# Yoshiki172/Deep-Learning-based-RGBA-Image-Compression-with-Masked-Window-based-Attention

Measured on AMD Instinct MI355X. Metric: MPixels/sec encode+decode, 256×256 RGBA batch; bpp & PSNR parity vs reference, higher is better.
Workload: dtype bf16; 1 GPU; AutoEncoderRGB_Journal forward encode+decode (BASELINE config 2), 256x256 RGBA; global_batch=8, per_gpu_batch=8, height=256, width=256, parallelism=replicas1, hip_graph=True, tile_cache=profiles/tune_fwd_bf16_b8_256.json

## Files before the change

### deep-learning-based-rgba-image-compression-with-masked-window-based-attention_amd/csrc/conv.hip

```cpp
#include <cstdio>
#include <cstdlib>
#include <utility>

#include "common.h"
#include "conv_common.h"

namespace rgbac {

#ifdef RGBAC_WG_TIMING
__device__ unsigned long long g_wg_t[16384][4];
#define WG_T(k)                                                                              \
  do {                                                                                       \
    if (threadIdx.x == 0) {                                                                  \
      const unsigned b_ = blockIdx.x + gridDim.x * (blockIdx.y + gridDim.y * blockIdx.z);    \
      if (b_ < 16384) g_wg_t[b_][k] = wall_clock64();                                        \
    }                                                                                        \
  } while (0)
#else
#define WG_T(k) do {} while (0)
#endif

template <typename T, int BM, int BN, int WGM, int WGN, int NBUF, int KSM = 1>
__global__ void __launch_bounds__(256) conv_kernel(const ConvArgsDev args) {
  constexpr int EPV = Elem<T>::EPV;
// ... 1935 lines not shown
#pragma unroll
          for (int r = 0; r < 4; ++r) v[j][r] += t[r];
        }
    }
#pragma unroll
    for (int j = 0; j < TN; ++j)
      if (nn[j] < cout) Elem<T>::st4(out + opix * ldo + nn[j], v[j]);
  }
}

template <int TN, int TM, bool DACT>
__device__ __forceinline__ void patch_epilogue(const ConvShared& s, const ConvGroup& g, int ph,
                                               int b, int yrow0, int x0, int fr,
                                               const int (&nn)[TN], const f32x4 (&acc)[TN][TM],
                                               const float (*pbias)[4] = nullptr) {
  const bool lean = s.mode != RGBAC_SUBPEL2 && !g.zout && !g.res1 && (g.cout & 3) == 0;
  if (lean && s.act == RGBAC_ACT_NONE) {
    patch_epi<TN, TM, RGBAC_ACT_NONE>(s, g, ph, b, yrow0, x0 + fr, nn, acc, pbias);
  } else if (lean && s.act == RGBAC_ACT_GELU) {
    patch_epi<TN, TM, RGBAC_ACT_GELU>(s, g, ph, b, yrow0, x0 + fr, nn, acc, pbias);
  } else if (lean && s.act == RGBAC_ACT_RELU) {
    patch_epi<TN, TM, RGBAC_ACT_RELU>(s, g, ph, b, yrow0, x0 + fr, nn, acc, pbias);
  } else if (DACT && lean && is_dact(s.act)) {
    patch_epi<TN, TM, RGBAC_ACT_DGELU>(s, g, ph, b, yrow0, x0 + fr, nn, acc, pbias);
  } else {
#pragma unroll
    for (int i = 0; i < TM; ++i) {
      const int m = (b * s.Hm + yrow0 + i) * s.Wm + x0 + fr;
      epilogue_tile_row<bf16_t, TN, TM, DACT>(s, g, ph, m, nn, acc, i);
    }
  }
}

template <int TH, int BN, int WGM, int WGN, int NBUF, bool DACT>
__global__ void __launch_bounds__(512) conv_patch_kernel(const ConvArgsDev args) {
  using T = bf16_t;
  constexpr int NW = 8;
  static_assert(WGM * WGN == NW, "8 waves");
  constexpr int TW = 16, PW = TW + 2, PH = TH + 2, PR = PH * PW;
  constexpr int RSC = 10;
  constexpr int PPIECE = (PR * RSC + 63) / 64;
  constexpr int PQ = (PPIECE + NW - 1) / NW;
  constexpr int TM = TH / WGM, TN = BN / WGN / 16;
  static_assert(TM >= 1 && TN >= 1 && TM * WGM == TH && TN * WGN * 16 == BN, "tile");
  constexpr int IA = BN / 8;
  constexpr int NAW = (IA + NW - 1) / NW;
  static_assert(NBUF == 3 || NBUF == 4, "ring depth (the patch rider sits at tap NBUF-1 of "
                                        "a group; groups have >= 4 taps)");
  constexpr int RT = NBUF - 1;
  constexpr int WSTAGE = BN * 8;
  constexpr int PSTAGE = PPIECE * 64;
  __shared__ __attribute__((aligned(16))) uint4 smem[NBUF * WSTAGE + 2 * PSTAGE];

  const ConvShared& s = args.s;
  const int tid = threadIdx.x, lane = tid & 63;
  const int wave = __builtin_amdgcn_readfirstlane(tid >> 6);
  const int txn = s.Wm / TW, tyn = s.Hm / TH;
  int nblk, txi, tyi, b, gi;
  {
    const int nwg = gridDim.x * gridDim.y;
    int t = blockIdx.x + gridDim.x * blockIdx.y;
    if (s.remap) {
      const int xcd = t & 7, q = nwg >> 3, r = nwg & 7;
      t = (xcd < r ? xcd * (q + 1) : r * (q + 1) + (xcd - r) * q) + (t >> 3);
    }
    nblk = t % gridDim.y; t /= gridDim.y;
    txi = t % txn; t /= txn;
// ... 153 lines not shown
    __builtin_amdgcn_s_barrier();
    __builtin_amdgcn_sched_barrier(0);
    if (it + NBUF - 1 < ns) STAGE_ISSUE(it + NBUF - 1);
    const uint4* As = smem + (it % NBUF) * WSTAGE;
    const uint4* Ps = smem + NBUF * WSTAGE + (cgrp & 1) * PSTAGE + toff;
#pragma unroll
    for (int ks = 0; ks < 2; ++ks) {
      uint4 a[TN], bb[TM];
#pragma unroll
      for (int j = 0; j < TN; ++j) a[j] = As[(ks ? a1 : a0) + j * 128];
#pragma unroll
      for (int i = 0; i < TM; ++i) bb[i] = Ps[bbase[i] + 4 * ks];
#pragma unroll
      for (int j = 0; j < TN; ++j)
#pragma unroll
        for (int i = 0; i < TM; ++i) mma_step<T>(acc[j][i], a[j], bb[i]);
    }
    ++ctap;
    if (++ctx == ctw) {
      ctx = 0;
      toff += convt ? (-PW + ctw - 1) * RSC : (PW - ctw + 1) * RSC;
    } else {
      toff += convt ? -RSC : RSC;
    }
    if (ctap == cntap) {
      ctap = 0; ctx = 0; ++cgrp;
      toff = convt ? (2 * PW + 2) * RSC : 0;
      if (++cck == nck) {
        cck = 0;
        if (!s2 || cph == 3 || pz >= 0) {
          int nn[TN];
#pragma unroll
          for (int j = 0; j < TN; ++j) nn[j] = n0 + wn * TN * 16 + j * 16 + fq * 4;
          if (s2 && pz >= 0) {
#pragma unroll
            for (int i = 0; i < TM; ++i) {
              const int m = (b * s.Hm + y0 + wm * TM + i) * s.Wm + x0 + fr;
#pragma unroll
              for (int j = 0; j < TN; ++j)
                if (nn[j] < g.cout)
                  *reinterpret_cast<float4*>(g.ws + ((size_t)pz * s.M + m) * g.cout16 + nn[j]) =
                      make_float4(acc[j][i][0], acc[j][i][1], acc[j][i][2], acc[j][i][3]);
            }
          } else {
            patch_epilogue<TN, TM, DACT>(s, g, s2 ? 0 : cph, b, y0 + wm * TM, x0, fr, nn, acc);
          }
#pragma unroll
          for (int j = 0; j < TN; ++j)
#pragma unroll
            for (int i = 0; i < TM; ++i) acc[j][i] = f32x4{0.f, 0.f, 0.f, 0.f};
        }
        ++cph;
        ctw = 3 - (cph & 1);
        cntap = (3 - (cph >> 1)) * ctw;
      }
    }
  }
#undef STAGE_ISSUE
#undef PATCH_ISSUE
}

template <int TH, int BN, int NW, int R, int CPT = 0, int KS = 1>
__global__ void __launch_bounds__(64 * NW * KS) conv_fpatch_kernel(const ConvArgsDev args) {
  using T = bf16_t;
  constexpr int TW = 16, PW = TW + 2, PR = (TH + 2) * PW;
  constexpr int TM = TH, TN = BN / NW / 16;
  static_assert(TN * NW * 16 == BN, "tile");
// ... 715 lines not shown
  if (tile < 0 || tile >= kNumTiles) return -1;
  return (fpatch_tile(tile) || kTiles[tile].kind == kNPatch) ? 1 : 0;
}
extern "C" int rgbac_conv_max_groups(void) { return kMaxGroups; }

extern "C" int rgbac_conv2d_grouped_describe(const rgbac_conv_args* args, int ngroups,
                                             char* kernel, int cap) {
  ConvArgsDev d;
  ConvPlan p;
  const int rc = plan_conv(args, ngroups, false, d, p);
  if (rc == RGBAC_OK && kernel && cap > 0) snprintf(kernel, (size_t)cap, "%s", p.name);
  return rc;
}

extern "C" int rgbac_conv2d_grouped(const rgbac_conv_args* args, int ngroups, void* stream) {
  return rgbac_conv2d_grouped_part(args, ngroups, 0, stream);
}

extern "C" int rgbac_conv2d_grouped_part(const rgbac_conv_args* args, int ngroups, int part,
                                         void* stream) {
  RGBAC_REQUIRE(part >= 0 && part <= 2, "part must be 0 (all), 1 (main) or 2 (split-K epilogue)");
  ConvArgsDev d;
  ConvPlan p;
  const int rc = plan_conv(args, ngroups, true, d, p);
  if (rc) return rc;
  hipStream_t st = reinterpret_cast<hipStream_t>(stream);
  if (args[0].dtype == RGBAC_F32) return launch_conv<float>(d, p, st, part);
  return launch_conv<bf16_t>(d, p, st, part);
}

extern "C" int rgbac_conv2d(const rgbac_conv_args* a, void* stream) {
  return rgbac_conv2d_grouped(a, 1, stream);
}
```

### deep-learning-based-rgba-image-compression-with-masked-window-based-attention_amd/csrc/conv_common.h

```cpp
#pragma once
#include "common.h"

namespace rgbac {

constexpr int kMaxGroups = 10;

struct ConvGroup {
  const void* sp0; const void* sp1; const void* sp2;
  long long sld0, sld1, sld2;
  const void* w;
  const float* bias;
  void* out;
  const void* res0; const void* res1; const void* res2;
  long long ld0, ld1, ld2, out_ldc;
  const uint8_t* sel;
  float* ws;
  const float* aux0;
  float* aux1;
  double* partial;
  void* zout;
  long long zld;
  int* cnt;
  int send0, send1, send2;
  int cin_pad, k_pad, cout, rows, cout16, out_coff;
// ... 374 lines not shown
    }
  }
}

template <typename T>
__device__ __forceinline__ float gauss_elem(const ConvGroup& g, int m, int c, int nch, float mu,
                                            float sg) {
  const float yv = Elem<T>::ld(reinterpret_cast<const T*>(g.res1) + (long long)m * g.ld1 + c);
  const float hat = rintf(yv - mu) + mu;
  Elem<T>::st(reinterpret_cast<T*>(g.out) + (long long)m * g.out_ldc + g.out_coff + c, hat);
  const float xin = g.aux0 ? yv + g.aux0[(long long)m * nch + c] : hat;
  const float v = fabsf(xin - mu);
  const float sc = fmaxf(sg, 0.11f);
  const float lik = fmaxf(std_cum_f((0.5f - v) / sc) - std_cum_f((-0.5f - v) / sc), 1e-9f);
  if (g.aux1) g.aux1[(long long)m * nch + c] = lik;
  const float bits = (-1.0f * logf(lik + 1e-10f)) / 0.69314718055994530942f;
  return fminf(fmaxf(bits, 0.0f), 50.0f);
}

template <typename T>
__device__ __forceinline__ float gauss_elem_y(const ConvGroup& g, int m, int c, int nch, float mu,
                                              float sg, float yv) {
  const float hat = rintf(yv - mu) + mu;
  Elem<T>::st(reinterpret_cast<T*>(g.out) + (long long)m * g.out_ldc + g.out_coff + c, hat);
  const float xin = g.aux0 ? yv + g.aux0[(long long)m * nch + c] : hat;
  const float v = fabsf(xin - mu);
  const float sc = fmaxf(sg, 0.11f);
  const float lik = fmaxf(std_cum_f((0.5f - v) / sc) - std_cum_f((-0.5f - v) / sc), 1e-9f);
  if (g.aux1) g.aux1[(long long)m * nch + c] = lik;
  const float bits = (-1.0f * logf(lik + 1e-10f)) / 0.69314718055994530942f;
  return fminf(fmaxf(bits, 0.0f), 50.0f);
}

bool pw3_ok(const ConvArgsDev& d, int cin_max);
void launch_pw3(const ConvArgsDev& d, hipStream_t st);

typedef __attribute__((address_space(3))) void* lptr_t;

__device__ __forceinline__ void dma16(const void* src, uint4* lds_block) {
  const uint32_t lds = __builtin_amdgcn_readfirstlane((uint32_t)(size_t)(lptr_t)lds_block);
  uint32_t keep;
  asm volatile(
      "s_mov_b32 %0, m0\n\t"
      "s_mov_b32 m0, %2\n\t"
      "s_nop 0\n\t"
      "global_load_lds_dwordx4 %1, off\n\t"
      "s_mov_b32 m0, %0"
      : "=&s"(keep)
      : "v"(src), "s"(lds)
      : "memory");
}

__device__ __forceinline__ void dma16_s(const void* sbase, uint32_t voff, uint32_t lds) {
  uint32_t keep;
  asm volatile(
      "s_mov_b32 %0, m0\n\t"
      "s_mov_b32 m0, %3\n\t"
      "s_nop 0\n\t"
      "global_load_lds_dwordx4 %1, %2\n\t"
      "s_mov_b32 m0, %0"
      : "=&s"(keep)
      : "v"(voff), "s"(sbase), "s"(lds)
      : "memory");
}
__device__ __forceinline__ void dma16_l(const void* src, uint32_t lds) {
  uint32_t keep;
// ... 31 lines not shown
```

### deep-learning-based-rgba-image-compression-with-masked-window-based-attention_amd/rgbac/_lib.py

```python
import ctypes
import os

import torch

_HERE = os.path.dirname(os.path.abspath(__file__))
LIB_PATH = os.environ.get("RGBAC_LIB_PATH") or os.path.join(_HERE, "librgbac_hip.so")

F32, BF16 = 0, 1
ACT = dict(none=0, gelu=1, relu=2, lrelu=3, tanh_half=4, gate=5, gdn=6, igdn=7, masksel=8,
           gauss=9, sqbwd=10, dgelu=11, dlrelu=12)
CONV, CONVT_S2, SUBPEL2 = 0, 1, 2
TILE_KINDS = ("stream", "deep", "pers", "wres", "direct", "spatial", "smallk", "wstream", "patch",
              "fpatch", "fpatch_ks", "pw", "npatch")


class Src(ctypes.Structure):
    _fields_ = [("ptr", ctypes.c_void_p), ("ldc", ctypes.c_int64),
                ("channels", ctypes.c_int32), ("_pad", ctypes.c_int32)]


class ConvArgs(ctypes.Structure):
    _fields_ = [
        ("dtype", ctypes.c_int32), ("mode", ctypes.c_int32),
        ("batch", ctypes.c_int32), ("in_h", ctypes.c_int32), ("in_w", ctypes.c_int32),
# ... 63 lines not shown
    "rgbac_conv_tile_info": [_I32, ctypes.POINTER(ctypes.c_int), ctypes.POINTER(ctypes.c_int),
                             ctypes.POINTER(ctypes.c_int)],
    "rgbac_conv2d_grouped": [ctypes.c_void_p, _I32, _VP],
    "rgbac_conv2d_grouped_part": [ctypes.c_void_p, _I32, _I32, _VP],
    "rgbac_conv2d_grouped_describe": [ctypes.c_void_p, _I32, ctypes.c_char_p, _I32],
    "rgbac_conv_max_groups": [],
    "rgbac_timer_create": [ctypes.POINTER(ctypes.c_void_p)],
    "rgbac_timer_record": [_VP, _VP],
    "rgbac_timer_elapsed_ms": [_VP, _VP, ctypes.POINTER(ctypes.c_float)],
    "rgbac_timer_destroy": [_VP],
    "rgbac_winattn_core": [_I32, _I32, _I32, _I32, _I32, _I32, _I32, _I32, _I32, _F,
                           _VP, _I64, _VP, _VP, _VP, _I64, _VP, _VP],
    "rgbac_winattn_core_ex": [_I32, _I32, _I32, _I32, _I32, _I32, _I32, _I32, _I32, _F,
                              _VP, _I64, _VP, _VP, _VP, _I64, _VP, _VP, _I32, _I32, _VP],
    "rgbac_gaussian_slice": [_I32, _I64, _I32, _VP, _I64, _VP, _I64, _VP, _I64, _VP,
                             _VP, _I64, _VP, _VP, _VP],
    "rgbac_eb_forward": [_I32, _I64, _I32, _VP, _I64, _VP, _VP, _VP, _I64, _VP, _VP, _VP],
    "rgbac_reduce_blocks": [_I64],
    "rgbac_finalize": [_I32, _I32, _I32, _I32, _I32, _I32, _VP, _VP, _I64, _VP, _VP, _I32,
                       _VP, _I32, _VP, _VP, _VP],
    "rgbac_finalize_blocks": [_I32, _I32],
    "rgbac_finalize_ex": [_I32, _I32, _I32, _I32, _I32, _I32, _VP, _VP, _I64, _VP, _VP, _I32,
                          _VP, _I32, _VP, _VP, _VP, _VP],
    "rgbac_forward_prologue": [_I32, _I32, _I32, _I32, _I32, _VP, _VP, _I64, _VP, _I32, _VP,
                               _I32, _VP, _VP, _I64, _VP],
    "rgbac_mask_pyramid": [_I32, _I32, _I32, _VP, _I32, _VP, _I32, _VP, _VP],
    "rgbac_nchw_to_nhwc": [_I32, _I32, _I32, _I32, _I32, _VP, _VP, _I64, _VP],
    "rgbac_nhwc_to_nchw": [_I32, _I32, _I32, _I32, _I32, _VP, _I64, _VP, _VP],
    "rgbac_residual_unit": [_VP, _I32, _VP],
    "rgbac_residual_unit_ex": [_VP, _I32, _I32, _VP],
    "rgbac_residual_unit_gate": [_VP, _VP, _VP, _VP, _I64, _VP, _I64, _VP],
    "rgbac_stem_gdn": [_I32, _I32, _I32, _VP, _I64, _VP, _I32, _VP, _VP, _I32, _VP, _I32, _VP,
                       _I64, _VP],
    "rgbac_winattn_block": [_I32, _I32, _I32, _I32, _I32, _F, _VP, _I64, _VP, _VP, _VP, _VP, _VP,
                            _VP, _I64, _VP, _I64, _VP],
    "rgbac_winattn_block_workspace": [_I32, _I32, _I32],
    "rgbac_gdn_reparam": [_I32, _I32, _VP, _VP, _F, _F, _F, _VP, _VP, _VP],
    "rgbac_gdn_reparam_bwd": [_I32, _I32, _VP, _VP, _F, _F, _VP, _VP, _VP, _VP, _I32, _VP],
    "rgbac_eb_params": [_I32, _VP, _VP, _VP],
    "rgbac_eb_params_bwd": [_I32, _VP, _VP, _VP, _I32, _VP],
    "rgbac_winattn_block_ws4": [_I32, _I32, _I32, _I32, _I32, _F, _VP, _I64, _VP, _VP, _VP, _VP,
                                _VP, _VP, _VP, _I64, _VP],
    "rgbac_rgba_augment": [_I32, _VP, _I32, _I32, _I32, _VP, _VP, _VP, _VP, _VP],
    "rgbac_dse_block": [_I32, _I32, _I32, _I32, _I32, _F, _VP, _I64, _VP, _I64, _VP, _I32, _VP, _VP,
                        _I32, _VP, _VP, _I32, _VP, _VP, _I32, _VP, _VP, _I64, _VP],
    "rgbac_act_bwd": [_I32, _I32, _F, _I64, _I32, _VP, _I64, _VP, _I64, _VP, _I64, _VP, _VP,
                      _I64, _VP, _I64, _VP],
    "rgbac_conv_wgrad": [ctypes.POINTER(WgradArgs), _VP],
    "rgbac_wgrad_reduce": [_I64, _VP, _VP, _I32, _I64, _VP, _I32, _VP, _I32, _VP, _I32, _VP],
    "rgbac_wgrad_reduce_multi": [_I32, _VP, _VP],
    "rgbac_winattn_core_bwd": [_I32, _I32, _I32, _I32, _I32, _I32, _I32, _I32, _I32, _F, _VP,
                               _I64, _VP, _VP, _VP, _I64, _VP, _I64, _I32, _VP, _VP],
    "rgbac_winattn_core_bwd_ex": [_I32, _I32, _I32, _I32, _I32, _I32, _I32, _I32, _I32, _F,
                                  _VP, _I64, _VP, _VP, _VP, _I64, _VP, _I64, _I32, _VP, _VP,
                                  _I32, _VP],
    "rgbac_relpos_bwd": [_I32, _I32, _I32, _VP, _VP, _VP, _VP, _VP, _VP],
    "rgbac_gaussian_bwd": [_I32, _I64, _I32, _VP, _I64, _VP, _I64, _VP, _I64, _VP, _VP, _VP,
                           _I64, _VP, _I64, _VP, _I64, _VP, _I64, _VP],
    "rgbac_eb_bwd": [_I32, _I64, _I32, _VP, _I64, _VP, _VP, _VP, _VP, _I64, _VP, _I64, _VP, _VP],
    "rgbac_mse_bwd": [_I32, _I32, _I32, _I32, _I32, _I32, _VP, _VP, _I64, _VP, _VP, _VP, _VP,
                      _I64, _VP],
    "rgbac_adam_clamp": [_I64, _VP, _VP, _VP, _VP, _D, _D, _D, _D, _I64, _F, _F, _VP],
    "rgbac_adam_clamp_dstep": [_I64, _VP, _VP, _VP, _VP, _D, _D, _D, _D, _VP, _F, _F, _VP],
    "rgbac_pixel_shuffle": [_I32, _I32, _I32, _I32, _I32, _I32, _VP, _I64, _VP, _I64, _VP],
    "rgbac_channel_copy": [_I32, _I64, _I32, _VP, _I64, _I32, _VP, _I64, _I32, _VP],
    "rgbac_channel_copy_multi": [_I32, _I64, _I32, _VP, _VP],
# ... 105 lines not shown
```

### deep-learning-based-rgba-image-compression-with-masked-window-based-attention_amd/rgbac/layers/TransformRGB.py

```python
import torch
import torch.nn as nn

from .. import runtime as rt
from .GDN import GDN
from .Masked_Attention import Win_noShift_Attention
from .masked_win_attention import needs_grad
from ._blocks import conv3x3, subpel_conv3x3


def _act_of(m):
    if isinstance(m, nn.LeakyReLU):
        return "lrelu", float(m.negative_slope)
    if isinstance(m, nn.ReLU):
        return "relu", 0.0
    if isinstance(m, nn.GELU):
        return "gelu", 0.0
    raise TypeError(f"unsupported activation {type(m)}")


def _layer_forward(module, nhwc_fn, train_fn, x):
    rt.check_gpu(x)
    if needs_grad(module, x):
        from .. import train_forward as tf
        fn = getattr(tf, train_fn)
        return tf.layer_t(lambda f: fn(module, f), x)
    with torch.no_grad():
        return rt.to_nchw(nhwc_fn(rt.to_nhwc(x, torch.float32)))


def run_conv(m, srcs, **kw):
    return rt.launch([prep_conv(m, srcs, **kw)])[0]


def prep_conv(m, srcs, **kw):
    dt = srcs[0][0].t.dtype
    segs = rt.segs_of(*srcs)
    if isinstance(m, nn.ConvTranspose2d):
        k, s = m.kernel_size[0], m.stride[0]
        if k == 1 and s == 1:
            pk = rt.packed(m, dt, segs, rt.CONV, transposed=True)
        elif m.out_channels <= 4:
            assert k == 5 and s == 2 and m.padding[0] == 2 and m.output_padding[0] == 1
            pk = rt.packed(m, dt, segs, rt.SUBPEL2, transposed=True)
        else:
            assert k == 5 and s == 2 and m.padding[0] == 2 and m.output_padding[0] == 1
            pk = rt.packed(m, dt, segs, rt.CONVT_S2)
    else:
        assert m.padding[0] == m.kernel_size[0] // 2 and m.dilation[0] == 1 and m.groups == 1
        pk = rt.packed(m, dt, segs)
    return rt.prepare(pk, srcs, **kw)


def prep_subpel(seq, srcs, act="none"):
    assert isinstance(seq[1], nn.PixelShuffle) and seq[1].upscale_factor == 2
    dt = srcs[0][0].t.dtype
    pk = rt.packed(seq[0], dt, rt.segs_of(*srcs), rt.SUBPEL2)
    return rt.prepare(pk, srcs, act=act)


def run_subpel(seq, srcs, act="none"):
    return rt.launch([prep_subpel(seq, srcs, act)])[0]


class EnhancementBlock(nn.Module):
    def __init__(self, num_filters=32):
        super().__init__()
        self.conv1 = nn.Conv2d(num_filters, num_filters, 3, stride=1, padding=1)
        self.relu = nn.ReLU(inplace=True)
        self.conv2 = nn.Conv2d(num_filters, num_filters, 3, stride=1, padding=1)

    def nhwc(self, x, post=None):
        act, slope = _act_of(self.relu)
        t = run_conv(self.conv1, [x.src()], act=act, act_param=slope)
        return run_conv(self.conv2, [t.src()], res0=x, res2=post)

    def forward(self, input):
        return _layer_forward(self, lambda f: self.nhwc(f), "enhancement_t", input)


def dse_fused_ok(dse, x):
    if not (rt.DSE_FUSED and x.t.dtype == torch.bfloat16 and x.C in (1, 3) and x.ldc % 8 == 0):
        return False
    if dse.input_conv.out_channels != 32:
# ... 63 lines not shown
class Analysis_transform(nn.Module):
    def __init__(self, N=192, M=320):
        super().__init__()
        self.x1 = nn.Conv2d(3, N, 5, stride=2, padding=2)
        self.gdn1 = GDN(N)
        self.x2 = nn.Conv2d(N, N, 5, stride=2, padding=2)
        self.gdn2 = GDN(N)
        self.attention1 = Win_noShift_Attention(dim=N, num_heads=8, window_size=8, shift_size=4)
        self.x3 = nn.Conv2d(N, N, 5, stride=2, padding=2)
        self.gdn3 = GDN(N)
        self.x4 = nn.Conv2d(N, M, 1, stride=1, padding=0)
        self.attention2 = Win_noShift_Attention(dim=M, num_heads=8, window_size=4, shift_size=2)

    def _stem(self, x):
        m = self.x1
        if (x.t.dtype == torch.bfloat16 and x.ldc == 8 and m.out_channels == 192 and
                m.kernel_size == (5, 5) and m.stride == (2, 2) and m.padding == (2, 2) and
                not self.gdn1.inverse and rt.STEM_FUSED):
            pk1 = rt.packed(m, x.t.dtype, rt.segs_of(x.src()))
            pk2 = self.gdn1._pack(x.t.dtype, 192)
            out = rt.new_feat(x.B, (x.H + 1) // 2, (x.W + 1) // 2, 192, x.t.dtype, x.t.device)
            rt.timed("stem_gdn_kernel", 2.0 * out.B * out.H * out.W * 192 * (75 + 192),
                     2.0 * (x.B * x.H * x.W * 8 + out.B * out.H * out.W * 192),
                     lambda: rt._lib.call("rgbac_stem_gdn", x.B, x.H, x.W, x.ptr(), x.ldc,
                                          pk1.w.data_ptr(), pk1.k_pad, pk1.bias.data_ptr(),
                                          pk2.w.data_ptr(), pk2.k_pad, pk2.bias.data_ptr(), 0,
                                          out.ptr(), out.ldc, rt._lib.stream_ptr(x.t.device)),
                     f"stem_gdn_kernel 3->192 {x.H}x{x.W} B{x.B}")
            return out
        return self.gdn1.nhwc(run_conv(m, [x.src()]))

    def nhwc(self, x, me2, me3):
        y = self._stem(x)
        y = self.gdn2.nhwc(run_conv(self.x2, [y.src()]))
        y = self.attention1.nhwc(y, me2)
        y = self.gdn3.nhwc(run_conv(self.x3, [y.src()]))
        y = run_conv(self.x4, [y.src()])
        return self.attention2.nhwc(y, me3)

    def forward(self, input, mask, me1, me2, me3, me4):
        rt.check_gpu(input, me2, me3)
        if needs_grad(self, input):
            from ..train_forward import analysis_t, layer_t
            return layer_t(lambda f: analysis_t(self, f, me2, me3), input)
        with torch.no_grad():
            return rt.to_nchw(self.nhwc(rt.to_nhwc(input, torch.float32), me2, me3))


class Synthesis_transform(nn.Module):
    def __init__(self, N=196, M=320):
        super().__init__()
        self.attention1 = Win_noShift_Attention(dim=M, num_heads=8, window_size=4, shift_size=2)
        self.x1 = nn.Conv2d(M, N, 1, stride=1, padding=0)
        self.igdn1 = GDN(N, inverse=True)
        self.x2 = nn.ConvTranspose2d(N, N, 5, stride=2, padding=2, output_padding=1)
        self.igdn2 = GDN(N, inverse=True)
        self.attention2 = Win_noShift_Attention(N, num_heads=8, window_size=8, shift_size=4)
        self.x3 = nn.ConvTranspose2d(N, N, 5, stride=2, padding=2, output_padding=1)
        self.igdn3 = GDN(N, inverse=True)
        self.x4 = nn.ConvTranspose2d(N, 3, 5, stride=2, padding=2, output_padding=1)
        self.dse = DSE(32)

    def nhwc(self, y, md2, md3):
        t = self.attention1.nhwc(y, md3)
        t = self.igdn1.nhwc(run_conv(self.x1, [t.src()]))
        t = self.igdn2.nhwc(run_conv(self.x2, [t.src()]))
        t = self.attention2.nhwc(t, md2)
        t = self.igdn3.nhwc(run_conv(self.x3, [t.src()]))
        x4o = rt.new_feat(t.B, 2 * t.H, 2 * t.W, self.x4.out_channels, t.t.dtype, t.t.device,
                          zero=False)
        if not dse_fused_ok(self.dse, x4o):
            x4o.t.zero_()
        t = run_conv(self.x4, [t.src()], out=x4o)
        return self.dse.nhwc(t)

    def forward(self, input, reconmask, md1, md2, md3, md4):
        rt.check_gpu(input, md2, md3)
        if needs_grad(self, input):
            from ..train_forward import layer_t, synthesis_t
            return layer_t(lambda f: synthesis_t(self, f, md2, md3), input)
        with torch.no_grad():
            return rt.to_nchw(self.nhwc(rt.to_nhwc(input, torch.float32), md2, md3))
```

### deep-learning-based-rgba-image-compression-with-masked-window-based-attention_amd/rgbac/runtime.py

```python
import contextlib
import ctypes
import json
import os

import torch

from . import _lib
from ._lib import ACT, CONV, CONVT_S2, SUBPEL2


PROFILER = None

PARAM_GEN = 0


class _Timer:
    __slots__ = ("h",)

    def __init__(self):
        h = ctypes.c_void_p()
        _lib.call("rgbac_timer_create", ctypes.byref(h))
        self.h = h

    def record(self):
# ... 100 lines not shown

def _patch_split_ok(preps):
    a = preps[0].a
    return (a.mode == CONVT_S2 or (a.mode == CONV and a.ksize == 5 and a.stride == 2)) and \
        a.act not in (ACT["dgelu"], ACT["dlrelu"])


def frag_weights(pk):
    f = getattr(pk, "frag", None)
    if f is not None:
        return f
    nph, rows, _ = pk.w.shape
    taps = 9 if pk.mode == CONVT_S2 else pk.ksize * pk.ksize
    cp, c32 = pk.cin_pad, round_up(pk.cin_pad, 32)
    w = pk.w[:, :, :taps * cp].reshape(nph, rows, taps, cp)
    wt = torch.zeros((nph, rows, taps, c32), dtype=pk.w.dtype, device=pk.w.device)
    wt[..., :cp] = w
    nks = taps * c32 // 32
    fr = wt.reshape(nph, rows // 16, 16, nks, 4, 8).permute(0, 1, 3, 4, 2, 5).contiguous()
    pk.frag = fr
    return fr


def _has_frag(pk):
    return isinstance(pk, PackedConv) or getattr(pk, "frag", None) is not None


KSPLITS = (1, 2, 4, 8)
TUNE = os.environ.get("RGBAC_TUNE", "1") != "0"
TILE_SET = os.environ.get("RGBAC_TILE_SET", "stream")
_tune_cache = {}
FORCE = None
STEM_FUSED = os.environ.get("RGBAC_STEM_FUSED", "1") != "0"
DSE_FUSED = os.environ.get("RGBAC_DSE_FUSED", "1") != "0"
WINBLOCK_FUSED = os.environ.get("RGBAC_WINBLOCK", "1") != "0"
WINBLOCK4_FUSED = os.environ.get("RGBAC_WINBLOCK4", "1") != "0"


_SIDE_STREAMS = {}
SIDE = os.environ.get("RGBAC_SIDE_STREAMS", "0") == "1"


def side_streams(dev):
    cur = torch.cuda.current_stream(dev)
    if not SIDE:
        return cur, cur
    st = _SIDE_STREAMS.get(dev)
    if st is None:
        st = _SIDE_STREAMS[dev] = torch.cuda.Stream(device=dev)
    return cur, st


def pick_cout_pad(cout):
    return round_up(cout, 128)


def _candidates(M, cout, nst, nks=None, plain=True, spatial=False, smallk=False, wstream=False):
    out = [(TILE_SMALLK, 1)] if smallk else []
    if wstream:
        out.append((TILE_WSTREAM, 1))
    n16 = round_up(cout, 16)
    for t, (bm, bn) in enumerate(TILES):
        if t in (TILE_SMALLK, TILE_WSTREAM) or t >= FIRST_PATCH:
            continue
        if t == TILE_SPATIAL:
            if spatial:
# ... 456 lines not shown
                        arr[i].out = outs[i]
                        for name in ("res0", "res1", "res2"):
                            if getattr(arr[i], name) == s_ptr:
                                setattr(arr[i], name, outs[i])
                torch.cuda.synchronize(dev)
                del scratch
        elif gauss:
            choice = min(candidates(preps), key=lambda c: TILES[c[0]][1])
        else:
            choice = _heuristic(mtot, cout, nst)
        if not fixed:
            _tune_cache[key] = choice
    choice = resolve_choice(choice, preps)
    set_choice(*choice)
    LAST_CHOICE[0] = tuple(choice)
    if PROFILER is None:
        run()
    else:
        name = kernel_name(choice[0], preps)
        desc = f"{name} ks{choice[1]} g{n} {p0.desc}"
        PROFILER.wrap(name, sum(pr.flops for pr in preps), sum(pr.nbytes for pr in preps),
                      lambda: _lib.call("rgbac_conv2d_grouped_part", ctypes.addressof(arr), n, 1,
                                        _lib.stream_ptr(dev)), desc)
        if choice[1] > 1 and not arr[0].tile_counters:
            dts = "float" if p0.a.dtype == 0 else "bf16_t"
            PROFILER.wrap(f"conv_splitk_epilogue<{dts}>", 0.0,
                          sum(4.0 * choice[1] * pr.mgrid * pr.nphase * pr.pk.cout for pr in preps),
                          lambda: _lib.call("rgbac_conv2d_grouped_part", ctypes.addressof(arr), n,
                                            2, _lib.stream_ptr(dev)),
                          f"conv_splitk_epilogue ks{choice[1]} g{n} {p0.desc}")
    return [pr.out for pr in preps]


def conv(pk, srcs, **kw):
    return launch([prepare(pk, srcs, **kw)])[0]


def feat_srcs(f):
    return [(f, 0, f.ldc)]


def packed(m, dtype, segs, mode=CONV, transposed=False, weight=None, bias=None):
    w = m.weight if weight is None else weight
    b = getattr(m, "bias", None) if bias is None else bias
    key = (dtype, tuple(segs), mode, transposed)
    ver = (PARAM_GEN, w._version, w.data_ptr(),
           None if b is None else (b._version, b.data_ptr()))
    cache = m.__dict__.setdefault("_rgbac_pack", {})
    ent = cache.get(key)
    if ent is None or ent[0] != ver:
        ww = w if w.dim() == 4 else w.reshape(w.shape[0], w.shape[1], 1, 1)
        stride = m.stride[0] if hasattr(m, "stride") else 1
        cache[key] = (ver, PackedConv(ww, b, mode, segs, dtype, stride=stride,
                                      transposed=transposed))
    return cache[key][1]


def segs_of(*srcs):
    out = []
    for f, coff, nch in srcs:
        if nch <= 0:
            continue
        real = min(nch, f.C - coff) if coff < f.C else 0
        out.append((real, nch))
    return out

# ... 7 lines not shown
```

### include/rgbac.h

```cpp
#ifndef RGBAC_H_
#define RGBAC_H_

#include <stdint.h>

#ifdef __cplusplus
extern "C" {
#endif

#define RGBAC_ABI_VERSION 2

enum rgbac_status {
  RGBAC_OK = 0,
  RGBAC_E_ARG = -1,
  RGBAC_E_DTYPE = -2,
  RGBAC_E_LAUNCH = -3,
};

enum rgbac_dtype { RGBAC_F32 = 0, RGBAC_BF16 = 1 };

enum rgbac_act {
  RGBAC_ACT_NONE = 0,
  RGBAC_ACT_GELU = 1,
  RGBAC_ACT_RELU = 2,
  RGBAC_ACT_LRELU = 3,
// ... 197 lines not shown

int rgbac_adam_clamp(int64_t n, float* param, float* grad, float* exp_avg, float* exp_avg_sq,
                     double lr, double beta1, double beta2, double eps, int64_t step,
                     float clip, float grad_scale, void* stream);

int rgbac_adam_clamp_dstep(int64_t n, float* param, float* grad, float* exp_avg,
                           float* exp_avg_sq, double lr, double beta1, double beta2, double eps,
                           int64_t* step_dev, float clip, float grad_scale, void* stream);

int rgbac_pixel_shuffle(int dtype, int dir, int batch, int h, int w, int c, const void* in,
                        int64_t ldi, void* out, int64_t ldo, void* stream);
int rgbac_channel_copy(int dtype, int64_t npix, int channels, const void* src, int64_t lds,
                       int scoff, void* dst, int64_t ldd, int dcoff, void* stream);
int rgbac_channel_copy_multi(int dtype, int64_t npix, int ntasks, const int64_t* desc,
                             void* stream);

int rgbac_channel_copy_multi_ex(int dtype, int64_t npix, int ntasks, const int64_t* desc,
                                void* stream);

int rgbac_weight_gather(int dtype, int64_t n, const float* src, const int32_t* idx, void* dst,
                        void* stream);

int rgbac_weight_gather_multi(int ntask, const int64_t* tasks, const int64_t* blk0, int64_t nblk,
                              void* stream);
int rgbac_weight_repack_multi(int ntask, const int64_t* tasks, const int64_t* blk0, int64_t nblk,
                              void* stream);
int rgbac_colsum(int dtype, int64_t npix, int channels, const void* x, int64_t ldx, int nsplit,
                 float* partial, void* stream);
int rgbac_sum_partials(int rows, int n, const double* partial, float* out, void* stream);

int rgbac_stem_gdn(int batch, int in_h, int in_w, const void* x, int64_t x_ldc, const void* w1,
                   int w1_kpad, const float* b1, const void* w2, int w2_kpad, const float* beta,
                   int inverse, void* out, int64_t out_ldc, void* stream);

int rgbac_rgba_augment(int batch, const void* descs, int out_h, int out_w, int antialias,
                       float* masked, float* alpha, float* img, float* rgba, void* stream);

int rgbac_gdn_reparam(int nb, int ng, const float* beta, const float* gamma, float beta_bound,
                      float gamma_bound, float pedestal, float* beta_out, float* gamma_out,
                      void* stream);
int rgbac_gdn_reparam_bwd(int nb, int ng, const float* beta, const float* gamma,
                          float beta_bound, float gamma_bound, const float* dbeta_out,
                          const float* dgamma_out, float* dbeta, float* dgamma, int accumulate,
                          void* stream);

int rgbac_eb_params(int channels, const float* const* params, float* out, void* stream);
int rgbac_eb_params_bwd(int channels, const float* const* params, const float* dout,
                        float* const* grads, int accumulate, void* stream);

int64_t rgbac_winattn_block_workspace(int batch, int h, int w);
int rgbac_winattn_block(int batch, int h, int w, int shift, int masked, float scale,
                        const void* x, int64_t ldx, const float* alpha, const void* wq_packed,
                        const float* bias_pack, const void* wp_packed, const float* table_pad,
                        void* out, int64_t ldo, void* work, int64_t work_bytes, void* stream);

int rgbac_winattn_block_ws4(int batch, int h, int w, int shift, int masked, float scale,
                            const void* x, int64_t ldx, const float* alpha, const void* wq_packed,
                            const float* bqkv, const void* wp_packed, const float* bproj,
                            const float* table, void* out, int64_t ldo, void* stream);

int rgbac_dse_block(int mode, int batch, int h, int w, int cin, float slope, const void* x,
                    int64_t ldx,
                    const void* t, int64_t ldt, const void* w_in, int kp_in, const float* b_in,
                    const void* w1, int kp1, const float* b1, const void* w2, int kp2,
                    const float* b2, const void* w_out, int kp_out, const float* b_out,
                    void* out, int64_t ldo, void* stream);
// ... 124 lines not shown
```

Baseline: 310.9 MPix/s.

## Fuse GDN/IGDN tail into the patch conv kernel epilogue for 192-channel convs

Adds a GDN template variant of the patch conv kernel. After accumulation it stages the conv output tile in a free LDS weight ring slot, runs the 192x192 gamma matmul on squared activations via MFMA, and applies GDN or IGDN before storing. This removes a separate GDN kernel launch plus the round trip of writing and re-reading the intermediate activation for three encoder/decoder layers. In exchange the epilogue holds gamma fragments in registers and adds a block sync, which may hurt occupancy. It only applies when the tuned tile is the 128x192 patch tile.

```diff
diff --git a/deep-learning-based-rgba-image-compression-with-masked-window-based-attention_amd/csrc/conv.hip b/deep-learning-based-rgba-image-compression-with-masked-window-based-attention_amd/csrc/conv.hip
--- a/deep-learning-based-rgba-image-compression-with-masked-window-based-attention_amd/csrc/conv.hip
+++ b/deep-learning-based-rgba-image-compression-with-masked-window-based-attention_amd/csrc/conv.hip
@@ -1991,7 +1991,7 @@
   }
 }
 
-template <int TH, int BN, int WGM, int WGN, int NBUF, bool DACT>
+template <int TH, int BN, int WGM, int WGN, int NBUF, bool DACT, bool GDN = false>
 __global__ void __launch_bounds__(512) conv_patch_kernel(const ConvArgsDev args) {
   using T = bf16_t;
   constexpr int NW = 8;
@@ -2211,7 +2211,55 @@
           int nn[TN];
 #pragma unroll
           for (int j = 0; j < TN; ++j) nn[j] = n0 + wn * TN * 16 + j * 16 + fq * 4;
-          if (s2 && pz >= 0) {
+          if constexpr (GDN) {
+            static_assert(!GDN || (BN == 192 && TM * 16 * 24 == WSTAGE), "GDN tail tile");
+            const int live = (ns - 1) % NBUF;
+            const int slot = wm == 0 ? (live == 0 ? 1 : 0)
+                                     : (live == NBUF - 1 ? NBUF - 2 : NBUF - 1);
+            uint4 ga[TN][6];
+            float gbeta[TN][4], gbias[TN][4];
+            const int c0 = wn * TN * 16;
+#pragma unroll
+            for (int j = 0; j < TN; ++j)
+#pragma unroll
+              for (int r = 0; r < 4; ++r)
+                gbias[j][r] = g.bias ? g.bias[c0 + 16 * j + 4 * fq + r] : 0.0f;
+            {
+              const bf16_t* const gw = reinterpret_cast<const bf16_t*>(g.res1);
+              const int gk = (int)g.ld1;
+#pragma unroll
+              for (int j = 0; j < TN; ++j) {
+                const bf16_t* const row = gw + (size_t)(c0 + 16 * j + fr) * gk + fq * 8;
+#pragma unroll
+                for (int st = 0; st < 6; ++st)
+                  ga[j][st] = *reinterpret_cast<const uint4*>(row + 32 * st);
+              }
+            }
+#pragma unroll
+            for (int j = 0; j < TN; ++j)
+#pragma unroll
+              for (int r = 0; r < 4; ++r) gbeta[j][r] = g.aux0[c0 + 16 * j + 4 * fq + r];
+            uint2 yq[TN][TM];
+#pragma unroll
+            for (int j = 0; j < TN; ++j)
+#pragma unroll
+              for (int i = 0; i < TM; ++i)
+                yq[j][i] = make_uint2(
+                    pack_bf16x2(acc[j][i][0] + gbias[j][0], acc[j][i][1] + gbias[j][1]),
+                    pack_bf16x2(acc[j][i][2] + gbias[j][2], acc[j][i][3] + gbias[j][3]));
+            gdn_tail<TN, TM>(smem + slot * WSTAGE, wn * TN * 16, fr, fq, yq, ga, gbeta, s.act);
+            const int py = convt ? cph >> 1 : 0, px = convt ? cph & 1 : 0, sc = convt ? 2 : 1;
+            bf16_t* const out = reinterpret_cast<bf16_t*>(g.out) + g.out_coff;
+#pragma unroll
+            for (int i = 0; i < TM; ++i) {
+              const long long opix =
+                  (long long)(b * s.out_h + sc * (y0 + wm * TM + i) + py) * s.out_w +
+                  sc * (x0 + fr) + px;
+#pragma unroll
+              for (int j = 0; j < TN; ++j)
+                *reinterpret_cast<uint2*>(out + opix * g.out_ldc + nn[j]) = yq[j][i];
+            }
+          } else if (s2 && pz >= 0) {
 #pragma unroll
             for (int i = 0; i < TM; ++i) {
               const int m = (b * s.Hm + y0 + wm * TM + i) * s.Wm + x0 + fr;
@@ -2993,3 +3041,43 @@
 extern "C" int rgbac_conv2d(const rgbac_conv_args* a, void* stream) {
   return rgbac_conv2d_grouped(a, 1, stream);
 }
+
+template <int NBUF>
+static void launch_patch_gdn(const ConvArgsDev& d, const ConvPlan& p, hipStream_t st) {
+  hipLaunchKernelGGL((conv_patch_kernel<8, 192, 2, 4, NBUF, false, true>), p.grid, dim3(512), 0,
+                     st, d);
+}
+
+extern "C" int rgbac_conv_gdn(const rgbac_conv_args* a, const void* gamma, int gamma_kpad,
+                              const float* beta, int inverse, void* stream) {
+  RGBAC_REQUIRE(a != nullptr, "null args");
+  RGBAC_REQUIRE(gamma && beta, "null gamma / beta");
+  RGBAC_REQUIRE(gamma_kpad >= 192 && gamma_kpad % 8 == 0 && ((uintptr_t)gamma % 16) == 0,
+                "the gamma pack needs k_pad >= 192, a multiple of 8, and 16-byte alignment");
+  RGBAC_REQUIRE(a->dtype == RGBAC_BF16, "the GDN tail is bf16 only");
+  RGBAC_REQUIRE(a->act == RGBAC_ACT_NONE, "the GDN tail takes a conv without activation");
+  RGBAC_REQUIRE(!a->res0 && !a->res1 && !a->res2 && !a->zout,
+                "the GDN tail takes a conv without residual or pre-activation store");
+  RGBAC_REQUIRE(a->cout == 192, "the GDN tail needs cout == 192");
+  RGBAC_REQUIRE(a->tile >= 0 && a->tile < kNumTiles, "tile index out of range");
+  const TileDesc tc = kTiles[a->tile];
+  RGBAC_REQUIRE(tc.kind == kPatch && tc.bm == 128 && tc.bn == 192 && tc.a == 2 && tc.b == 4 &&
+                    (tc.c == 3 || tc.c == 4),
+                "the GDN tail runs on the conv_patch_kernel tiles with bn = 192");
+  RGBAC_REQUIRE((a->mode == RGBAC_CONV && a->ksize == 5 && a->stride == 2 && a->ksplit == 1) ||
+                    (a->mode == RGBAC_CONVT_S2 && a->ksplit == 4),
+                "the GDN tail needs the unsplit 5x5/s2 conv or the phase-split convT");
+  RGBAC_REQUIRE(a->out_ldc >= a->out_coff + 192, "out_ldc too small for the 192 channels");
+  ConvArgsDev d;
+  ConvPlan p;
+  const int rc = plan_conv(a, 1, true, d, p);
+  if (rc) return rc;
+  d.s.act = inverse ? RGBAC_ACT_IGDN : RGBAC_ACT_GDN;
+  d.g[0].res1 = gamma;
+  d.g[0].ld1 = gamma_kpad;
+  d.g[0].aux0 = beta;
+  hipStream_t st = reinterpret_cast<hipStream_t>(stream);
+  if (tc.c == 3) launch_patch_gdn<3>(d, p, st);
+  else launch_patch_gdn<4>(d, p, st);
+  return check_launch("conv_patch_kernel<gdn>");
+}
diff --git a/deep-learning-based-rgba-image-compression-with-masked-window-based-attention_amd/csrc/conv_common.h b/deep-learning-based-rgba-image-compression-with-masked-window-based-attention_amd/csrc/conv_common.h
--- a/deep-learning-based-rgba-image-compression-with-masked-window-based-attention_amd/csrc/conv_common.h
+++ b/deep-learning-based-rgba-image-compression-with-masked-window-based-attention_amd/csrc/conv_common.h
@@ -430,6 +430,53 @@
   return fminf(fmaxf(bits, 0.0f), 50.0f);
 }
 
+template <int TN, int TM>
+__device__ __forceinline__ void gdn_tail(uint4* X, int cw, int fr, int fq, uint2 (&yq)[TN][TM],
+                                         const uint4 (&ga)[TN][6], const float (&beta)[TN][4],
+                                         int act) {
+  constexpr int TS = 24;
+#pragma unroll
+  for (int j = 0; j < TN; ++j) {
+    const int c = (cw + 16 * j + 4 * fq) >> 3;
+#pragma unroll
+    for (int i = 0; i < TM; ++i)
+      *reinterpret_cast<uint2*>(reinterpret_cast<char*>(X + (i * 16 + fr) * TS + (c ^ (fr & 7))) +
+                                8 * (fq & 1)) = yq[j][i];
+  }
+  __syncthreads();
+  f32x4 acc[TN][TM];
+#pragma unroll
+  for (int j = 0; j < TN; ++j)
+#pragma unroll
+    for (int i = 0; i < TM; ++i) acc[j][i] = f32x4{0.f, 0.f, 0.f, 0.f};
+#pragma unroll
+  for (int st = 0; st < 6; ++st) {
+    uint4 b[TM];
+#pragma unroll
+    for (int i = 0; i < TM; ++i)
+      b[i] = square_chunk<bf16_t>(X[(i * 16 + fr) * TS + ((4 * st + fq) ^ (fr & 7))]);
+#pragma unroll
+    for (int j = 0; j < TN; ++j)
+#pragma unroll
+      for (int i = 0; i < TM; ++i) mma_step<bf16_t>(acc[j][i], ga[j][st], b[i]);
+  }
+#pragma unroll
+  for (int j = 0; j < TN; ++j)
+#pragma unroll
+    for (int i = 0; i < TM; ++i) {
+      const uint2 q = yq[j][i];
+      const float x4[4] = {bf2f(q.x & 0xFFFF), bf2f(q.x >> 16), bf2f(q.y & 0xFFFF),
+                           bf2f(q.y >> 16)};
+      float v[4];
+#pragma unroll
+      for (int r = 0; r < 4; ++r) {
+        const float nrm = acc[j][i][r] + beta[j][r];
+        v[r] = act == RGBAC_ACT_GDN ? gdn_t<bf16_t>(x4[r], nrm) : igdn_t<bf16_t>(x4[r], nrm);
+      }
+      yq[j][i] = make_uint2(pack_bf16x2(v[0], v[1]), pack_bf16x2(v[2], v[3]));
+    }
+}
+
 bool pw3_ok(const ConvArgsDev& d, int cin_max);
 void launch_pw3(const ConvArgsDev& d, hipStream_t st);
 
diff --git a/deep-learning-based-rgba-image-compression-with-masked-window-based-attention_amd/rgbac/_lib.py b/deep-learning-based-rgba-image-compression-with-masked-window-based-attention_amd/rgbac/_lib.py
--- a/deep-learning-based-rgba-image-compression-with-masked-window-based-attention_amd/rgbac/_lib.py
+++ b/deep-learning-based-rgba-image-compression-with-masked-window-based-attention_amd/rgbac/_lib.py
@@ -119,6 +119,7 @@
     "rgbac_residual_unit_gate": [_VP, _VP, _VP, _VP, _I64, _VP, _I64, _VP],
     "rgbac_stem_gdn": [_I32, _I32, _I32, _VP, _I64, _VP, _I32, _VP, _VP, _I32, _VP, _I32, _VP,
                        _I64, _VP],
+    "rgbac_conv_gdn": [ctypes.POINTER(ConvArgs), _VP, _I32, _VP, _I32, _VP],
     "rgbac_winattn_block": [_I32, _I32, _I32, _I32, _I32, _F, _VP, _I64, _VP, _VP, _VP, _VP, _VP,
                             _VP, _I64, _VP, _I64, _VP],
     "rgbac_winattn_block_workspace": [_I32, _I32, _I32],
diff --git a/deep-learning-based-rgba-image-compression-with-masked-window-based-attention_amd/rgbac/layers/TransformRGB.py b/deep-learning-based-rgba-image-compression-with-masked-window-based-attention_amd/rgbac/layers/TransformRGB.py
--- a/deep-learning-based-rgba-image-compression-with-masked-window-based-attention_amd/rgbac/layers/TransformRGB.py
+++ b/deep-learning-based-rgba-image-compression-with-masked-window-based-attention_amd/rgbac/layers/TransformRGB.py
@@ -49,6 +49,16 @@
         assert m.padding[0] == m.kernel_size[0] // 2 and m.dilation[0] == 1 and m.groups == 1
         pk = rt.packed(m, dt, segs)
     return rt.prepare(pk, srcs, **kw)
+
+
+def conv_then_gdn(m, gdn, x):
+    if rt.GDN_FUSED and x.t.dtype == torch.bfloat16 and m.out_channels == 192:
+        pr = prep_conv(m, [x.src()])
+        choice = rt.gdn_tail_choice(pr)
+        if choice is not None:
+            return rt.conv_gdn(pr, gdn._pack(x.t.dtype, 192), gdn.inverse, choice)
+        return gdn.nhwc(rt.launch([pr])[0])
+    return gdn.nhwc(run_conv(m, [x.src()]))
 
 
 def prep_subpel(seq, srcs, act="none"):
@@ -178,9 +188,9 @@
 
     def nhwc(self, x, me2, me3):
         y = self._stem(x)
-        y = self.gdn2.nhwc(run_conv(self.x2, [y.src()]))
+        y = conv_then_gdn(self.x2, self.gdn2, y)
         y = self.attention1.nhwc(y, me2)
-        y = self.gdn3.nhwc(run_conv(self.x3, [y.src()]))
+        y = conv_then_gdn(self.x3, self.gdn3, y)
         y = run_conv(self.x4, [y.src()])
         return self.attention2.nhwc(y, me3)
 
@@ -210,7 +220,7 @@
     def nhwc(self, y, md2, md3):
         t = self.attention1.nhwc(y, md3)
         t = self.igdn1.nhwc(run_conv(self.x1, [t.src()]))
-        t = self.igdn2.nhwc(run_conv(self.x2, [t.src()]))
+        t = conv_then_gdn(self.x2, self.igdn2, t)
         t = self.attention2.nhwc(t, md2)
         t = self.igdn3.nhwc(run_conv(self.x3, [t.src()]))
         x4o = rt.new_feat(t.B, 2 * t.H, 2 * t.W, self.x4.out_channels, t.t.dtype, t.t.device,
diff --git a/deep-learning-based-rgba-image-compression-with-masked-window-based-attention_amd/rgbac/runtime.py b/deep-learning-based-rgba-image-compression-with-masked-window-based-attention_amd/rgbac/runtime.py
--- a/deep-learning-based-rgba-image-compression-with-masked-window-based-attention_amd/rgbac/runtime.py
+++ b/deep-learning-based-rgba-image-compression-with-masked-window-based-attention_amd/rgbac/runtime.py
@@ -156,6 +156,7 @@
 _tune_cache = {}
 FORCE = None
 STEM_FUSED = os.environ.get("RGBAC_STEM_FUSED", "1") != "0"
+GDN_FUSED = os.environ.get("RGBAC_GDN_FUSED", "1") != "0"
 DSE_FUSED = os.environ.get("RGBAC_DSE_FUSED", "1") != "0"
 WINBLOCK_FUSED = os.environ.get("RGBAC_WINBLOCK", "1") != "0"
 WINBLOCK4_FUSED = os.environ.get("RGBAC_WINBLOCK4", "1") != "0"
@@ -678,6 +679,43 @@
     return [pr.out for pr in preps]
 
 
+def gdn_tail_choice(pr):
+    if pr.a.dtype != _lib.BF16 or pr.pk.cout != 192 or pr.a.act != ACT["none"]:
+        return None
+    fixed = _FIXED[0] > 0
+    choice = None if fixed else (FORCE or _tune_cache.get(f"{pr.key}/g1"))
+    if choice is None:
+        if TUNE and not fixed and not torch.cuda.is_current_stream_capturing():
+            return None
+        choice = _heuristic(pr.mgrid * pr.nphase, pr.pk.cout, pr.nst)
+    t, ks = resolve_choice(choice, [pr])
+    if t not in PATCH_SIG or TILES[t] != (128, 192):
+        return None
+    if not ((pr.a.mode == CONV and pr.pk.ksize == 5 and pr.pk.stride == 2 and ks == 1) or
+            (pr.a.mode == CONVT_S2 and ks == 4)):
+        return None
+    return t, ks
+
+
+def conv_gdn(pr, gpk, inverse, choice):
+    t, ks = choice
+    a = pr.a
+    a.tile, a.ksplit = t, ks
+    a.workspace = a.tile_counters = None
+    a.weight = pr.pk.w.data_ptr()
+    o = pr.out
+    name = desc = "conv_patch_kernel"
+    if PROFILER is not None:
+        name = kernel_name(t, [pr]).replace("false>", "false, true>")
+        desc = f"{name} ks{ks} g1 {pr.desc} + {'igdn' if inverse else 'gdn'}"
+    LAST_CHOICE[0] = (t, ks)
+    timed(name, pr.flops + 2.0 * o.B * o.H * o.W * 192 * 192, pr.nbytes + gpk.w.numel() * 2,
+          lambda: _lib.call("rgbac_conv_gdn", ctypes.byref(a), gpk.w.data_ptr(), gpk.k_pad,
+                            gpk.bias.data_ptr(), 1 if inverse else 0,
+                            _lib.stream_ptr(o.t.device)), desc)
+    return o
+
+
 def conv(pk, srcs, **kw):
     return launch([prepare(pk, srcs, **kw)])[0]
 
diff --git a/include/rgbac.h b/include/rgbac.h
--- a/include/rgbac.h
+++ b/include/rgbac.h
@@ -253,6 +253,9 @@
 int rgbac_stem_gdn(int batch, int in_h, int in_w, const void* x, int64_t x_ldc, const void* w1,
                    int w1_kpad, const float* b1, const void* w2, int w2_kpad, const float* beta,
                    int inverse, void* out, int64_t out_ldc, void* stream);
+
+int rgbac_conv_gdn(const rgbac_conv_args* a, const void* gamma, int gamma_kpad, const float* beta,
+                   int inverse, void* stream);
 
 int rgbac_rgba_augment(int batch, const void* descs, int out_h, int out_w, int antialias,
                        float* masked, float* alpha, float* img, float* rgba, void* stream);
```

Measured after the change: 311.1 MPix/s, median of 3. About the same (+0.0%).
